# s-elkazdadi/ddp-pinocchio

Hardware: AMD Instinct MI355X
Metric: DDP iterations/sec (fwd+bwd sweep), Talos nq=38 T=200 (higher is better)
Workload: dtype f64

## Files before the change

ddp_pinocchio_amd/csrc/lin_static.hip:

```cpp
#include <float.h>
#include <math.h>
#include <stdlib.h>

#include <type_traits>
#include <utility>

#include "internal.h"
#include "lin_common.h"
#include "rbd.h"

#ifndef DEV_NO_EMIT
#define DEV_NO_EMIT 0
#endif
namespace {

struct TopoTalos38 {
  static constexpr int N = 38;
  static constexpr int parent[N] = {-1, 0, 1, 2, 3, 4,
                                    5, 6, 7, 8, 9, 10,
                                    5, 12, 13, 14, 15, 16,
                                    5, 18,
                                    19, 20, 21, 22, 23, 24, 25, 26,
                                    19, 28, 29, 30, 31, 32, 33, 34,
                                    19, 36};
  static constexpr int prismatic[N] = {1, 1, 1, 0, 0, 0, 0, 0, 0, 0, 0, 0, 0, 0, 0, 0, 0, 0, 0,
                                       0, 0, 0, 0, 0, 0, 0, 0, 0, 0, 0, 0, 0, 0, 0, 0, 0, 0, 0};
};

struct TopoChain6 {
  static constexpr int N = 6;
  static constexpr int parent[N] = {-1, 0, 1, 2, 3, 4};
  static constexpr int prismatic[N] = {0, 0, 0, 0, 0, 0};
};

}
#include "topo_extra.h"
namespace {

template <class T> constexpr bool has_child(int k) {
  for (int c = k + 1; c < T::N; ++c) if (T::parent[c] == k) return true;
  return false;
}
template <class T> constexpr int largest_child(int k) {
  int r = -1;
  for (int c = k + 1; c < T::N; ++c) if (T::parent[c] == k) r = c;
  return r;
}
template <class T> constexpr bool first_contrib(int k) { return T::parent[k] >= 0 && largest_child<T>(T::parent[k]) == k; }

template <class T>
bool topo_matches(const DevModel& m) {
  if (m.kind != DDP_HIP_MODEL_TREE || m.nv != T::N) return false;
  for (int i = 0; i < T::N; ++i)
    if (m.parent[i] != T::parent[i] || (m.jtype[i] == DDP_HIP_JOINT_PRISMATIC) != (T::prismatic[i] != 0)) return false;
  return true;
}

template <class T>
struct TauState {
  double acc[T::N][6];
  double uu[T::N];
};

template <class T, int K, int QS>
__device__ __forceinline__ void tau_up(const DevModel& m, const double* __restrict__ qc, const double* __restrict__ vc,
                                       double tauK, TauState<T>& s) {
  constexpr int o = T::prismatic[K] ? 3 : 0;
  const double* E = qc + K * QS;
  const double* r = E + 9;
  const double* U = E + 12;
  const double dinv = E[18];
  const double* pA0 = vc + K * rbd::VC_STRIDE + 6;
  const double* Iac = vc + K * rbd::VC_STRIDE + 12;
  const double* a = m.axis[K];
  double pAi[6];
  if constexpr (has_child<T>(K)) {
#pragma unroll
    for (int k = 0; k < 6; ++k) pAi[k] = s.acc[K][k];
  } else {
#pragma unroll
    for (int k = 0; k < 6; ++k) pAi[k] = pA0[k];
  }
  double sp = 0;
#pragma unroll
  for (int k = 0; k < 3; ++k) sp += a[k] * pAi[o + k];
  const double ui = tauK - sp;
  s.uu[K] = ui;
  constexpr int par = T::parent[K];
  if constexpr (par >= 0) {
    double pa[6], fp[6];
#pragma unroll
    for (int k = 0; k < 6; ++k) pa[k] = pAi[k] + Iac[k] + U[k] * (ui * dinv);
    rbd::xform_force_T(E, r, pa, fp);
    if constexpr (first_contrib<T>(K)) {
      const double* pp0 = vc + par * rbd::VC_STRIDE + 6;
#pragma unroll
      for (int k = 0; k < 6; ++k) s.acc[par][k] = pp0[k] + fp[k];
    } else {
#pragma unroll
      for (int k = 0; k < 6; ++k) s.acc[par][k] += fp[k];
    }
  }
  if constexpr (QS == rbd::QC_STRIDE || (K % 2) == 0) __builtin_amdgcn_sched_barrier(0);
}

template <class T, int K, int QS>
__device__ __forceinline__ void tau_down(const DevModel& m, const double* __restrict__ qc, const double* __restrict__ vc,
                                         TauState<T>& s) {
  constexpr int o = T::prismatic[K] ? 3 : 0;
  const double* E = qc + K * QS;
  const double* r = E + 9;
  const double* U = E + 12;
  const double dinv = E[18];
  const double* cb = vc + K * rbd::VC_STRIDE;
  double ap[6];
  constexpr int par = T::parent[K];
  if constexpr (par >= 0) rbd::xform_motion(E, r, s.acc[par], ap);
  else {
    const double a0[6] = {0, 0, 0, -m.gravity[0], -m.gravity[1], -m.gravity[2]};
    rbd::xform_motion(E, r, a0, ap);
  }
  double sum = 0;
#pragma unroll
  for (int k = 0; k < 6; ++k) { ap[k] += cb[k]; sum += U[k] * ap[k]; }
  const double qd = (s.uu[K] - sum) * dinv;
  s.uu[K] = qd;
  if constexpr (has_child<T>(K)) {
    const double* a = m.axis[K];
#pragma unroll
    for (int k = 0; k < 6; ++k) s.acc[K][k] = ap[k];
    s.acc[K][o] += a[0] * qd; s.acc[K][o + 1] += a[1] * qd; s.acc[K][o + 2] += a[2] * qd;
  }
  if constexpr (QS == rbd::QC_STRIDE || (K % 2) == 0) __builtin_amdgcn_sched_barrier(0);
}

template <class T, int QS, class TauFn, int... Ks>
__device__ __forceinline__ void tau_up_all(const DevModel& m, const double* __restrict__ qc, const double* __restrict__ vc, TauFn tau,
                                           TauState<T>& s, std::integer_sequence<int, Ks...>) {
  (tau_up<T, T::N - 1 - Ks, QS>(m, qc, vc, tau(T::N - 1 - Ks), s), ...);
}
template <class T, int QS, int HI, class TauFn, int... Ks>
__device__ __forceinline__ void tau_up_range(const DevModel& m, const double* __restrict__ qc, const double* __restrict__ vc, TauFn tau,
                                             TauState<T>& s, std::integer_sequence<int, Ks...>) {
  (tau_up<T, HI - Ks, QS>(m, qc, vc, tau(HI - Ks), s), ...);
}
template <class T, int QS, int... Ks>
__device__ __forceinline__ void tau_down_all(const DevModel& m, const double* __restrict__ qc, const double* __restrict__ vc,
                                             TauState<T>& s, std::integer_sequence<int, Ks...>) {
  (tau_down<T, Ks, QS>(m, qc, vc, s), ...);
}

constexpr int PS = 20;
template <int NV>
__device__ __forceinline__ void stage_placements(double* sp, const double* __restrict__ qc, int lane) {
  for (int idx = lane; idx < NV * 19; idx += LBS) {
    const int K = idx / 19, e = idx - K * 19;
    sp[K * PS + e] = qc[K * rbd::QC_STRIDE + e];
  }
}

template <int BYTES>
__device__ __forceinline__ unsigned int warm_block(const double* base, int lane) {
  typedef unsigned int u4 __attribute__((ext_vector_type(4)));
  const char* b = reinterpret_cast<const char*>(base);
  unsigned int sink = 0;
#pragma unroll
  for (int off = 0; off < BYTES; off += LBS * 16) {
    int o = off + lane * 16;
    o = o < BYTES - 16 ? o : BYTES - 16;
    const u4 v = *reinterpret_cast<const u4*>(b + o);
    sink ^= v.x ^ v.y ^ v.z ^ v.w;
  }
  return sink;
}

template <class T> constexpr bool parents_at_least(int from, int lo) {
  for (int k = from; k < T::N; ++k) if (T::parent[k] < lo) return false;
  return true;
}
template <class T> constexpr int stage_split() {
  for (int kh = T::N / 2; kh > 0; --kh) if (parents_at_least<T>(kh + 1, kh)) return kh;
  return 0;
}

template <int NV, int K0, int K1, bool WITH_V = true>
struct StageRegs {
  static constexpr int NPW = (K1 - K0) * 19, NVW = WITH_V ? (K1 - K0) * rbd::VC_STRIDE : 0;
  static constexpr int CP = (NPW + LBS - 1) / LBS, CV = (NVW + LBS - 1) / LBS;
  double rp[CP], rv[CV > 0 ? CV : 1];
  __device__ __forceinline__ void load(const double* __restrict__ qc, const double* __restrict__ vc, int lane) {
#pragma unroll
    for (int c = 0; c < CP; ++c) {
      int idx = c * LBS + lane;
      idx = idx < NPW ? idx : NPW - 1;
      const int K = K0 + idx / 19, e = idx % 19;
      rp[c] = qc[K * rbd::QC_STRIDE + e];
    }
#pragma unroll
    for (int c = 0; c < CV; ++c) {
      int idx = c * LBS + lane;
      idx = idx < NVW ? idx : NVW - 1;
      rv[c] = vc[K0 * rbd::VC_STRIDE + idx];
    }
  }
  __device__ __forceinline__ void park(double* sp, double* sv, int lane) const {
#pragma unroll
    for (int c = 0; c < CP; ++c) {
      int idx = c * LBS + lane;
      idx = idx < NPW ? idx : NPW - 1;
      const int K = K0 + idx / 19, e = idx % 19;
      sp[K * PS + e] = rp[c];
    }
#pragma unroll
    for (int c = 0; c < CV; ++c) {
      int idx = c * LBS + lane;
      idx = idx < NVW ? idx : NVW - 1;
      sv[K0 * rbd::VC_STRIDE + idx] = rv[c];
    }
  }
};

__device__ __forceinline__ void tri_index(int64_t q, int Wd, int& ii, int& jj) {
  int a = (int)floor(((2.0 * Wd - 1.0) - sqrt((2.0 * Wd - 1.0) * (2.0 * Wd - 1.0) - 8.0 * (double)q)) * 0.5);
  if (a < 0) a = 0;
  while ((int64_t)a * (2 * Wd - a - 1) / 2 > q) --a;
  while ((int64_t)(a + 1) * (2 * Wd - a - 2) / 2 <= q) ++a;
  ii = a;
  jj = (int)(q - (int64_t)a * (2 * Wd - a - 1) / 2) + a + 1;
}

template <int NV, int NP = LBS>
struct OutStage {
  double qdd[NP * (NV + 1)];
  int pij[NP];
};

template <int NV, int NP>
__device__ __forceinline__ void offdiag_emit(const LinParams& p, OutStage<NV, NP>& S, bool valid, int i, int j, int64_t bt,
                                             const double* __restrict__ xg, double dt, int pass = 0) {
  constexpr int n = 2 * NV, mm = NV;
  constexpr int RW = 16, NJ = (n + RW - 1) / RW, GRP = LBS / RW, PPG = NP / GRP, NB = NP == LBS ? 2 : 1;
  static_assert(PPG % NB == 0, "points per group");
  const double eps = sqrt(sqrt(DBL_EPSILON));
  const double eps2 = eps * eps;
  const int lane = threadIdx.x;
  if (lane / NP == pass) S.pij[lane % NP] = i | (j << 8) | ((valid ? 1 : 0) << 16);
  double* const fxx = p.fxx + bt * n * n * n;
  double* const fux = p.fux + bt * n * mm * n;
  double* const fuu = p.fuu + bt * n * mm * mm;
  const double* const fxb = p.fx + bt * n * n;
  const double* const fub = p.fu + bt * n * mm;
  __syncthreads();
  const int kk = lane % RW, grp = lane / RW;
  const double* f0 = p.f_val + bt * n;
  double f0k[NJ], xk[NJ], xvk[NJ];
#pragma unroll
  for (int jx = 0; jx < NJ; ++jx) {
    const int k = kk + RW * jx;
    const int kc = k < n ? k : n - 1;
    f0k[jx] = f0[kc];
    xk[jx] = xg[kc];
    xvk[jx] = kc < NV ? xg[NV + kc] : 0.0;
  }
  if (DEV_NO_EMIT) return;
  for (int pt = 0; pt < PPG; pt += NB) {
    double a1[NB][NJ], a2[NB][NJ], d1[NB][NJ], d2[NB][NJ];
    double* o0[NB];
    double* o1[NB];
    int ie[NB], je[NB], ee[NB];
#pragma unroll
    for (int u = 0; u < NB; ++u) {
      const int e = (pt + u) * GRP + grp;
      ee[u] = e;
      const int pk = S.pij[e];
      const int i1 = pk & 255, j1 = (pk >> 8) & 255;
      ie[u] = i1;
      je[u] = j1;
      const bool at_x_1 = i1 < n, at_x_2 = j1 < n;
      const int idx_1 = at_x_1 ? i1 : i1 - n, idx_2 = at_x_2 ? j1 : j1 - n;
      double* tensor;
      int L;
      if (at_x_1) { if (at_x_2) { tensor = fxx; L = n; } else { tensor = fux; L = mm; } }
      else { tensor = fuu; L = mm; }
      o0[u] = (pk >> 16) ? tensor + (int64_t)idx_2 * n + (int64_t)idx_1 * n * L : nullptr;
      o1[u] = ((pk >> 16) && at_x_1 == at_x_2 && !p.skip_qv_mirror) ? tensor + (int64_t)idx_1 * n + (int64_t)idx_2 * n * L : nullptr;
      if (o0[u]) {
        const double* q0 = at_x_1 ? fxb + (int64_t)idx_1 * n : fub + (int64_t)idx_1 * n;
        const double* q1 = at_x_2 ? fxb + (int64_t)idx_2 * n : fub + (int64_t)idx_2 * n;
        const double* q2 = at_x_1 ? fxx + (int64_t)idx_1 * n + (int64_t)idx_1 * n * n : fuu + (int64_t)idx_1 * n + (int64_t)idx_1 * n * mm;
        const double* q3 = at_x_2 ? fxx + (int64_t)idx_2 * n + (int64_t)idx_2 * n * n : fuu + (int64_t)idx_2 * n + (int64_t)idx_2 * n * mm;
#pragma unroll
        for (int jx = 0; jx < NJ; ++jx) {
          const int k = kk + RW * jx;
          const int kc = k < n ? k : n - 1;
          a1[u][jx] = q0[kc]; a2[u][jx] = q1[kc]; d1[u][jx] = q2[kc]; d2[u][jx] = q3[kc];
        }
      }
    }
#pragma unroll
    for (int u = 0; u < NB; ++u) {
      if (!o0[u]) continue;
#pragma unroll
      for (int jx = 0; jx < NJ; ++jx) {
        const int k = kk + RW * jx;
        if (k >= n) continue;
        if (p.skip_top && k < NV && !((ie[u] < n && ie[u] % NV == k) || (je[u] < n && je[u] % NV == k))) continue;
        double xs = k == ie[u] ? xk[jx] + eps : xk[jx];
        if (k == je[u]) xs = xs + eps;
        double fv;
        if (k < NV) {
          double xv = (NV + k) == ie[u] ? xvk[jx] + eps : xvk[jx];
          if (NV + k == je[u]) xv = xv + eps;
          const double vo = dt * xv;
          fv = xs + vo;
        } else {
          fv = xs + S.qdd[ee[u] * (NV + 1) + (k - NV)] * dt;
        }
        double df = fv - f0k[jx];
        df -= eps * a1[u][jx];
        df -= eps * a2[u][jx];
        df *= 2;
        const double val = 0.5 * (df / eps2 - d1[u][jx] - d2[u][jx]);
        o0[u][k] = val;
        if (o1[u]) o1[u][k] = val;
      }
    }
  }
}

template <int NV>
struct RowStage {
  double q[(NV + 2) * (NV + 1)];
};

template <int NV, bool DIAG_ROW, class ST>
__device__ __forceinline__ void rowblock_emit(const ST& S, int lane, int i, int jb, double* __restrict__ out, double* __restrict__ mirror,
                                              int64_t mstride, const double* __restrict__ a2, const double* __restrict__ d2, int64_t dstride,
                                              double dt, const double* __restrict__ f0g, const double* __restrict__ a1g,
                                              double* __restrict__ d1g, const double* __restrict__ xg, bool skip_top = false) {
  constexpr int n = 2 * NV, RW = 16, NJ = (n + RW - 1) / RW, CG = LBS / RW, NIT = (NV + CG - 1) / CG;
  const int r1 = i % NV;
  const double eps = sqrt(sqrt(DBL_EPSILON));
  const double eps2 = eps * eps;
  const int kk = lane % RW, cg = lane / RW;
  double xk[NJ], xvk[NJ], f0k[NJ], a1k[NJ], d1k[NJ];
#pragma unroll
  for (int j = 0; j < NJ; ++j) {
    const int k = kk + RW * j;
    const int kc = k < n ? k : n - 1;
    f0k[j] = f0g[kc];
    a1k[j] = a1g[kc];
    double x = xg[kc];
    if (kc == i) x = x + eps;
    xk[j] = x;
    double xv = xg[kc < NV ? NV + kc : kc];
    if (NV + kc == i) xv = xv + eps;
    xvk[j] = xv;
    if constexpr (DIAG_ROW) {
      double fv;
      if (kc < NV) {
        const double vo = dt * xv;
        fv = x + vo;
      } else {
        fv = x + S.q[NV * (NV + 1) + (kc - NV)] * dt;
      }
      double df = fv - f0k[j];
      df -= eps * a1k[j];
      df *= 2;
      const double dd = df / eps2;
      d1k[j] = dd;
      if (cg == 0 && k < n && !(skip_top && k < NV && k != r1)) d1g[k] = dd;
    } else {
      d1k[j] = d1g[kc];
    }
  }
  double va2[2][NJ], vd2[2][NJ];
  auto fetch = [&](int it, double (&A)[NJ], double (&D)[NJ]) {
    const int c = it * CG + cg;
    const int cc = c < NV ? c : NV - 1;
#pragma unroll
    for (int j = 0; j < NJ; ++j) {
      const int k = kk + RW * j;
      const int kc = k < n ? k : n - 1;
      A[j] = a2[kc + cc * n];
      D[j] = d2[kc + cc * dstride];
    }
  };
  auto form = [&](int it, const double (&A)[NJ], const double (&D)[NJ]) {
    const int c = it * CG + cg;
    const bool cv = c < NV;
    const int cc = cv ? c : NV - 1;
    const int jp = jb + cc;
#pragma unroll
    for (int j = 0; j < NJ; ++j) {
      const int k = kk + RW * j;
      if (!(cv && k < n)) continue;
      if (skip_top && k < NV && k != r1 && !(jp < n && jp % NV == k)) continue;
      double x = xk[j];
      if (k == jp) x = x + eps;
      double fv;
      if (k < NV) {
        double xv = xvk[j];
        if (NV + k == jp) xv = xv + eps;
        const double vo = dt * xv;
        fv = x + vo;
      } else {
        fv = x + S.q[cc * (NV + 1) + (k - NV)] * dt;
      }
      double df = fv - f0k[j];
      df -= eps * a1k[j];
      df -= eps * A[j];
      df *= 2;
      const double val = 0.5 * (df / eps2 - d1k[j] - D[j]);
      out[k + c * n] = val;
      if (mirror) mirror[k + c * mstride] = val;
    }
  };
  if (DEV_NO_EMIT) return;
  fetch(0, va2[0], vd2[0]);
  for (int it = 0; it < NIT; it += 2) {
    if (it + 1 < NIT) fetch(it + 1, va2[1], vd2[1]);
    form(it, va2[0], vd2[0]);
    if (it + 1 < NIT) {
      if (it + 2 < NIT) fetch(it + 2, va2[0], vd2[0]);
      form(it + 1, va2[1], vd2[1]);
    }
  }
}

template <class T, bool ROWS>
__global__ __launch_bounds__(LBS, ROWS ? 1 : 3) void lin_static_tau_kernel(LinParams p) {
  constexpr int nv = T::N, n = 2 * nv;
  constexpr int TRI = nv * (nv - 1) / 2, GU = (TRI + LBS - 1) / LBS, G = ROWS ? 2 * nv : GU;
  const int64_t bt = blockIdx.x / G;
  const int g = (int)(blockIdx.x % G) + (ROWS ? 0 : 2 * nv);
  const int lane = threadIdx.x;
  const int64_t Tn = p.d.T;
  const int b = (int)(bt / Tn);
  const int64_t t = bt % Tn;
  const DevModel& m = *p.model;
  int i, j, cfg, vcfg;
  bool valid;
  if (g < nv) { i = g; j = n + lane; cfg = 1 + g; vcfg = nv + 1 + g; valid = lane < nv; }
  else if (g < 2 * nv) { i = g; j = n + lane; cfg = 0; vcfg = 1 + (g - nv); valid = lane < nv; }
  else {
    const int pid = (g - 2 * nv) * LBS + lane;
    valid = pid < TRI;
    tri_index(valid ? pid : 0, nv, i, j);
    i += n; j += n; cfg = 0; vcfg = 0;
  }
  double eps = sqrt(sqrt(DBL_EPSILON));
  const double* __restrict__ qc = p.qcache + (bt * (nv + 1) + cfg) * (int64_t)nv * rbd::QC_STRIDE;
  const double* __restrict__ vc = p.vcache + (bt * (2 * nv + 1) + vcfg) * (int64_t)nv * rbd::VC_STRIDE;
  const double* __restrict__ xg = p.x + ((int64_t)b * (Tn + 1) + t) * n;
  const double* __restrict__ ug = p.u + ((int64_t)b * Tn + t) * nv;
  const int iu = i - n, ju = j - n;
  __shared__ union TauLds { double P[ROWS ? nv * PS + nv * rbd::VC_STRIDE : 1]; RowStage<nv> S; } s_lds;
  double* s_P = s_lds.P;
  unsigned int w = 0;
  double* s_V = s_P + nv * PS;
  constexpr int KH = ROWS ? stage_split<T>() : 0;
  StageRegs<nv, 0, (ROWS && KH > 0) ? KH : 1> lower;
  if constexpr (ROWS) {
    StageRegs<nv, KH, nv> upper;
    upper.load(qc, vc, lane);
    lower.load(qc, vc, lane);
    upper.park(s_P, s_V, lane);
    rbd::coop_sync<true>();
  } else {
    w = warm_block<nv * rbd::VC_STRIDE * 8>(vc, lane);
    w ^= warm_block<nv * rbd::QC_STRIDE * 8>(qc, lane);
  }
  if (w == 0x7fc01234u) eps = 0.0;
  TauState<T> s;
  auto tau = [&](int k) { double v = ug[k]; if (k == iu) v = v + eps; if (k == ju) v = v + eps; return v; };
  if constexpr (ROWS) {
    static_assert(!ROWS || parents_at_least<T>(KH + 1, KH), "the first half of the pass must not reach below record KH");
    tau_up_range<T, PS, nv - 1>(m, s_P, s_V, tau, s, std::make_integer_sequence<int, nv - 1 - KH>{});
    lower.park(s_P, s_V, lane);
    rbd::coop_sync<true>();
    tau_up_range<T, PS, KH>(m, s_P, s_V, tau, s, std::make_integer_sequence<int, KH + 1>{});
    tau_down_all<T, PS>(m, s_P, s_V, s, std::make_integer_sequence<int, nv>{});
  } else {
    tau_up_all<T, rbd::QC_STRIDE>(m, qc, vc, tau, s, std::make_integer_sequence<int, nv>{});
    tau_down_all<T, rbd::QC_STRIDE>(m, qc, vc, s, std::make_integer_sequence<int, nv>{});
  }
  __builtin_amdgcn_sched_barrier(0);
  typedef __attribute__((address_space(4))) const LinParams* kernarg_t;
  const kernarg_t kp = (kernarg_t)__builtin_amdgcn_kernarg_segment_ptr();
  if constexpr (ROWS) {
    RowStage<nv>& S = s_lds.S;
    const int mm = nv;
    __syncthreads();
    const int row = lane <= nv ? lane : nv + 1;
#pragma unroll
    for (int k = 0; k < nv; ++k) S.q[row * (nv + 1) + k] = s.uu[k];
    __syncthreads();
    rowblock_emit<nv, true>(S, lane, i, n, kp->fux + bt * n * mm * n + (int64_t)i * n * mm, nullptr, 0, kp->fu + bt * n * mm,
                            kp->fuu + bt * n * mm * mm, (int64_t)n + (int64_t)n * mm, m.dt, kp->f_val + bt * n,
                            kp->fx + bt * n * n + (int64_t)i * n, kp->fxx + bt * n * n * n + (int64_t)i * n + (int64_t)i * n * n, xg, kp->skip_top != 0);
  } else {
    __shared__ OutStage<nv, LBS / 2> S;
    LinParams po;
    po.f_val = kp->f_val; po.fx = kp->fx; po.fu = kp->fu; po.fxx = kp->fxx; po.fux = kp->fux; po.fuu = kp->fuu; po.skip_qv_mirror = kp->skip_qv_mirror; po.skip_top = kp->skip_top;
    const double dt = m.dt;
#pragma unroll 1
    for (int pass = 0; pass < 2; ++pass) {
      if (pass) __syncthreads();
      if (lane / (LBS / 2) == pass) {
#pragma unroll
        for (int k = 0; k < nv; ++k) S.qdd[(lane % (LBS / 2)) * (nv + 1) + k] = s.uu[k];
      }
      offdiag_emit<nv, LBS / 2>(po, S, valid, i, j, bt, xg, dt, pass);
    }
  }
}

template <class T> constexpr int n_children(int k) {
  int c = 0;
  for (int j = k + 1; j < T::N; ++j) if (T::parent[j] == k) ++c;
  return c;
}
template <class T> constexpr bool chain_start(int k) { return T::parent[k] < 0 || T::parent[k] != k - 1 || n_children<T>(T::parent[k]) > 1; }
template <class T> constexpr bool chain_end(int k) { return k == T::N - 1 || chain_start<T>(k + 1); }
template <class T> constexpr int chain_first(int k) { while (!chain_start<T>(k)) --k; return k; }
template <class T> constexpr int max_chain() {
  int best = 1;
  for (int k = 0; k < T::N; ++k)
    if (chain_end<T>(k)) { const int len = k - chain_first<T>(k) + 1; if (len > best) best = len; }
  return best;
}

template <class T>
struct VelState {
  double vel[T::N][6];
  double acc[T::N][6];
  double uu[T::N];
};

template <int UQS_, int QS_ = rbd::QC_STRIDE>
struct VelCtx {
  static constexpr int UQS = UQS_;
  static constexpr int QS = QS_;
  const DevModel* m;
  const double* qp;
  const double* __restrict__ qc;
  const double* __restrict__ xg;
  const double* __restrict__ ug;
  double* uq;
  int i, j;
  double eps;
  template <int K> __device__ __forceinline__ const double* er(double*) const { return qp + K * QS; }
  template <int K> __device__ __forceinline__ const double* er_down(double* b) const { return er<K>(b); }
  template <int K> __device__ __forceinline__ const double* ud() const { return qp + K * QS + 12; }
  template <int K> __device__ __forceinline__ void ia_cb(const double*, const double* cb, double* Iac) const { rbd::sym6_mv(qc + K * rbd::QC_STRIDE + 19, cb, Iac); }
  template <int K> __device__ __forceinline__ const double* ud_down() const { return ud<K>(); }
};

template <int NV, class C>
__device__ __forceinline__ double lane_v(const C& c, int K) {
  double v = c.xg[NV + K];
  if (NV + K == c.i) v = v + c.eps;
  if (NV + K == c.j) v = v + c.eps;
  return v;
}

template <class T, int K, class C>
__device__ __forceinline__ void joint_vel(const C& c, const double* vel_par, double* vel) {
  constexpr int o = T::prismatic[K] ? 3 : 0;
  double Pb[12];
  const double* E = c.template er<K>(Pb);
  const double* r = E + 9;
  const double* a = c.m->axis[K];
  const double vK = lane_v<T::N>(c, K);
  double vJ[6] = {0, 0, 0, 0, 0, 0};
  vJ[o] = a[0] * vK; vJ[o + 1] = a[1] * vK; vJ[o + 2] = a[2] * vK;
  if constexpr (T::parent[K] >= 0) rbd::xform_motion(E, r, vel_par, vel);
  else {
#pragma unroll
    for (int k = 0; k < 6; ++k) vel[k] = 0.0;
  }
#pragma unroll
  for (int k = 0; k < 6; ++k) vel[k] += vJ[k];
}
template <class T, int K, class C>
__device__ __forceinline__ void vel_from_root(const C& c, double* vel) {
  if constexpr (T::parent[K] >= 0) {
    double vp[6];
    vel_from_root<T, T::parent[K]>(c, vp);
    joint_vel<T, K>(c, vp, vel);
  } else {
    joint_vel<T, K>(c, nullptr, vel);
  }
}
template <class T, int K, class C>
__device__ __forceinline__ void bias_force0(const C& c, const double* vel, double* pA) {
  double Iv[6];
  rbd::sym6_mv(c.m->I6[K], vel, Iv);
  rbd::crf(vel, Iv, pA);
}

template <class T, int K, int E, class C>
__device__ __forceinline__ void chain_down(const C& c, VelState<T>& s) {
  if constexpr (T::parent[K] >= 0) joint_vel<T, K>(c, s.vel[T::parent[K]], s.vel[K]);
  else joint_vel<T, K>(c, nullptr, s.vel[K]);
  __builtin_amdgcn_sched_barrier(0);
  if constexpr (K < E) chain_down<T, K + 1, E>(c, s);
}

template <class T, int K, int F, class C>
__device__ __forceinline__ void chain_up(const C& c, VelState<T>& s) {
  constexpr int o = T::prismatic[K] ? 3 : 0;
  double Pb[12];
  const double* E = c.template er<K>(Pb);
  const double* r = E + 9;
  const double* U = c.template ud<K>();
  const double dinv = U[6];
  const double* a = c.m->axis[K];
  double pAi[6];
  if constexpr (has_child<T>(K)) {
#pragma unroll
    for (int k = 0; k < 6; ++k) pAi[k] = s.acc[K][k];
  } else {
    bias_force0<T, K>(c, s.vel[K], pAi);
  }
  double sp = 0;
#pragma unroll
  for (int k = 0; k < 3; ++k) sp += a[k] * pAi[o + k];
  const double ui = c.ug[K] - sp;
  if constexpr (C::UQS == 0) s.uu[K] = ui; else c.uq[K * C::UQS] = ui;
  constexpr int par = T::parent[K];
  if constexpr (par >= 0) {
    const double vK = lane_v<T::N>(c, K);
    double vJ[6] = {0, 0, 0, 0, 0, 0}, cb[6], pa[6], Iac[6], fp[6];
    vJ[o] = a[0] * vK; vJ[o + 1] = a[1] * vK; vJ[o + 2] = a[2] * vK;
    rbd::crm(s.vel[K], vJ, cb);
    c.template ia_cb<K>(U, cb, Iac);
#pragma unroll
    for (int k = 0; k < 6; ++k) pa[k] = pAi[k] + Iac[k] + U[k] * (ui * dinv);
    rbd::xform_force_T(E, r, pa, fp);
    if constexpr (first_contrib<T>(K)) {
      double p0[6];
      bias_force0<T, par>(c, s.vel[par], p0);
#pragma unroll
      for (int k = 0; k < 6; ++k) s.acc[par][k] = p0[k] + fp[k];
    } else {
#pragma unroll
      for (int k = 0; k < 6; ++k) s.acc[par][k] += fp[k];
    }
  }
  __builtin_amdgcn_sched_barrier(0);
  if constexpr (K > F) chain_up<T, K - 1, F>(c, s);
}

template <class T, int K, class C>
__device__ __forceinline__ void chain_at(const C& c, VelState<T>& s) {
  if constexpr (chain_end<T>(K)) {
    constexpr int F = chain_first<T>(K), P = T::parent[F];
    if constexpr (P >= 0) {
      if constexpr (first_contrib<T>(F) && n_children<T>(P) > 1) vel_from_root<T, P>(c, s.vel[P]);
    }
    chain_down<T, F, K>(c, s);
    chain_up<T, K, F>(c, s);
  }
}
template <class T, class C, int... Ks>
__device__ __forceinline__ void vel_up_all(const C& c, VelState<T>& s, std::integer_sequence<int, Ks...>) {
  (chain_at<T, T::N - 1 - Ks>(c, s), ...);
}

template <class T, int K, class C>
__device__ __forceinline__ void vel_down(const C& c, VelState<T>& s) {
  constexpr int o = T::prismatic[K] ? 3 : 0;
  constexpr int par = T::parent[K];
  double Pb[12];
  const double* E = c.template er_down<K>(Pb);
  const double* r = E + 9;
  const double* U = c.template ud_down<K>();
  const double dinv = U[6];
  const double* a = c.m->axis[K];
  const double vK = lane_v<T::N>(c, K);
  double vJ[6] = {0, 0, 0, 0, 0, 0}, vel[6], cb[6], ap[6];
  vJ[o] = a[0] * vK; vJ[o + 1] = a[1] * vK; vJ[o + 2] = a[2] * vK;
  if constexpr (par >= 0) {
    rbd::xform_motion(E, r, s.vel[par], vel);
    rbd::xform_motion(E, r, s.acc[par], ap);
  } else {
    const double a0[6] = {0, 0, 0, -c.m->gravity[0], -c.m->gravity[1], -c.m->gravity[2]};
#pragma unroll
    for (int k = 0; k < 6; ++k) vel[k] = 0.0;
    rbd::xform_motion(E, r, a0, ap);
  }
#pragma unroll
  for (int k = 0; k < 6; ++k) vel[k] += vJ[k];
  rbd::crm(vel, vJ, cb);
  double sum = 0;
#pragma unroll
  for (int k = 0; k < 6; ++k) { ap[k] += cb[k]; sum += U[k] * ap[k]; }
  double ui;
  if constexpr (C::UQS == 0) ui = s.uu[K]; else ui = c.uq[K * C::UQS];
  const double qd = (ui - sum) * dinv;
  if constexpr (C::UQS == 0) s.uu[K] = qd; else c.uq[K * C::UQS] = qd;
  if constexpr (has_child<T>(K)) {
#pragma unroll
    for (int k = 0; k < 6; ++k) { s.vel[K][k] = vel[k]; s.acc[K][k] = ap[k]; }
    s.acc[K][o] += a[0] * qd; s.acc[K][o + 1] += a[1] * qd; s.acc[K][o + 2] += a[2] * qd;
  }
  __builtin_amdgcn_sched_barrier(0);
}
template <class T, class C, int... Ks>
__device__ __forceinline__ void vel_down_all(const C& c, VelState<T>& s, std::integer_sequence<int, Ks...>) {
  (vel_down<T, Ks>(c, s), ...);
}

template <class T, bool ROWS>
__global__ __launch_bounds__(LBS, ROWS ? 3 : 1) void lin_static_vel_kernel(LinParams p) {
  constexpr int nv = T::N, n = 2 * nv;
  constexpr int TRI = nv * (nv - 1) / 2, GU = (TRI + LBS - 1) / LBS, G = ROWS ? nv : GU;
  const int64_t bt = blockIdx.x / G;
  const int g = (int)(blockIdx.x % G);
  const int lane = threadIdx.x;
  const int64_t Tn = p.d.T;
  const int b = (int)(bt / Tn);
  const int64_t t = bt % Tn;
  int i, j, cfg;
  bool valid;
  if (ROWS) { i = g; j = nv + lane; cfg = 1 + g; valid = lane < nv; }
  else {
    const int pid = g * LBS + lane;
    valid = pid < TRI;
    tri_index(valid ? pid : 0, nv, i, j);
    i += nv; j += nv; cfg = 0;
  }
  using Stage = typename std::conditional<ROWS, RowStage<nv>, OutStage<nv>>::type;
  __shared__ union VelLds { Stage S; double P[ROWS ? nv * rbd::QC_STRIDE : 1]; } s_lds;
  Stage& S = s_lds.S;
  double* s_P = s_lds.P;
  VelCtx<ROWS ? 0 : 1, rbd::QC_STRIDE> c;
  c.m = p.model;
  c.qc = p.qcache + (bt * (nv + 1) + cfg) * (int64_t)nv * rbd::QC_STRIDE;
  c.qp = ROWS ? s_P : c.qc;
  c.xg = p.x + ((int64_t)b * (Tn + 1) + t) * n;
  c.ug = p.u + ((int64_t)b * Tn + t) * nv;
  c.i = i; c.j = j;
  c.eps = sqrt(sqrt(DBL_EPSILON));
  if constexpr (ROWS) c.uq = nullptr;
  else c.uq = &S.qdd[lane * (nv + 1)];
  if constexpr (ROWS) {
    constexpr int NW = nv * rbd::QC_STRIDE, CW = (NW + LBS - 1) / LBS;
    double rq[CW];
#pragma unroll
    for (int r = 0; r < CW; ++r) { const int idx = r * LBS + lane; rq[r] = c.qc[idx < NW ? idx : NW - 1]; }
#pragma unroll
    for (int r = 0; r < CW; ++r) { const int idx = r * LBS + lane; s_P[idx < NW ? idx : NW - 1] = rq[r]; }
    c.qc = s_P;
    rbd::coop_sync<true>();
  } else {
    const unsigned int w = warm_block<nv * rbd::QC_STRIDE * 8>(c.qc, lane);
    if (w == 0x7fc01234u) c.eps = 0.0;
  }
  VelState<T> s;
  vel_up_all<T>(c, s, std::make_integer_sequence<int, nv>{});
  vel_down_all<T>(c, s, std::make_integer_sequence<int, nv>{});
  __builtin_amdgcn_sched_barrier(0);
  typedef __attribute__((address_space(4))) const LinParams* kernarg_t;
  const kernarg_t kp = (kernarg_t)__builtin_amdgcn_kernarg_segment_ptr();
  const double dt = c.m->dt;
  if constexpr (ROWS) {
    double* fxx = kp->fxx + bt * n * n * n;
    const double* fxb = kp->fx + bt * n * n;
    __syncthreads();
    const int row = valid ? lane : nv;
#pragma unroll
    for (int k = 0; k < nv; ++k) S.q[row * (nv + 1) + k] = s.uu[k];
    __syncthreads();
    rowblock_emit<nv, false>(S, lane, i, nv, fxx + (int64_t)nv * n + (int64_t)i * n * n,
                             kp->skip_qv_mirror ? nullptr : fxx + (int64_t)i * n + (int64_t)nv * n * n, (int64_t)n * n,
                             fxb + (int64_t)nv * n, fxx + (int64_t)nv * n + (int64_t)nv * n * n, (int64_t)n + (int64_t)n * n, dt,
                             kp->f_val + bt * n, fxb + (int64_t)i * n, fxx + (int64_t)i * n + (int64_t)i * n * n, c.xg, kp->skip_top != 0);
  } else {
    LinParams po;
    po.f_val = kp->f_val; po.fx = kp->fx; po.fu = kp->fu; po.fxx = kp->fxx; po.fux = kp->fux; po.fuu = kp->fuu; po.skip_qv_mirror = kp->skip_qv_mirror; po.skip_top = kp->skip_top;
    offdiag_emit<nv, LBS>(po, S, valid, i, j, bt, c.xg, dt);
  }
}

constexpr int WS_PER_JOINT = 8;

template <class T>
struct CfgState {
  double vel[T::N][6];
  double accP[T::N][6];
  double accI[T::N][21];
  double w[2][WS_PER_JOINT];
};

struct CfgCtx {
  const DevModel* __restrict__ m;
  const double* __restrict__ qc0;
  const double* __restrict__ xg;
  const double* __restrict__ ug;
  double* __restrict__ W;
  double* lvel;
  int i, j;
  const double* own;
};

template <int K, int NV>
__device__ __forceinline__ void lane_placement(const CfgCtx& c, double* P) {
  const double* base = c.qc0 + K * rbd::QC_STRIDE;
  const double* pert = c.own ? c.own : c.qc0 + ((int64_t)(1 + K) * NV + K) * rbd::QC_STRIDE;
  const bool own = K == c.i || K == c.j;
#pragma unroll
  for (int e = 0; e < 12; ++e) P[e] = own ? pert[e] : base[e];
}

template <class T, int K>
__device__ __forceinline__ void cfg_joint_vel(const CfgCtx& c, const double* P, const double* vel_par, double* vel) {
  constexpr int o = T::prismatic[K] ? 3 : 0;
  const double* a = c.m->axis[K];
  const double vK = c.xg[T::N + K];
  double vJ[6] = {0, 0, 0, 0, 0, 0};
  vJ[o] = a[0] * vK; vJ[o + 1] = a[1] * vK; vJ[o + 2] = a[2] * vK;
  if constexpr (T::parent[K] >= 0) rbd::xform_motion(P, P + 9, vel_par, vel);
  else {
#pragma unroll
    for (int k = 0; k < 6; ++k) vel[k] = 0.0;
  }
#pragma unroll
  for (int k = 0; k < 6; ++k) vel[k] += vJ[k];
}
template <class T, int K>
__device__ __forceinline__ void cfg_vel_from_root(const CfgCtx& c, double* vel) {
  double P[12];
  lane_placement<K, T::N>(c, P);
  if constexpr (T::parent[K] >= 0) {
    double vp[6];
    cfg_vel_from_root<T, T::parent[K]>(c, vp);
    cfg_joint_vel<T, K>(c, P, vp, vel);
  } else {
    cfg_joint_vel<T, K>(c, P, nullptr, vel);
  }
}
template <int K>
__device__ __forceinline__ void cfg_bias_force0(const CfgCtx& c, const double* vel, double* pA) {
  double Iv[6];
  rbd::sym6_mv(c.m->I6[K], vel, Iv);
  rbd::crf(vel, Iv, pA);
}

template <class T, int K, int F, int E>
__device__ __forceinline__ void cfg_chain_down(const CfgCtx& c, CfgState<T>& s, double* cur) {
  double P[12], vel[6];
  lane_placement<K, T::N>(c, P);
  if constexpr (T::parent[K] >= 0) cfg_joint_vel<T, K>(c, P, cur, vel);
  else cfg_joint_vel<T, K>(c, P, nullptr, vel);
#pragma unroll
  for (int k = 0; k < 6; ++k) { cur[k] = vel[k]; c.lvel[((K - F) * 6 + k) * LBS] = vel[k]; }
  __builtin_amdgcn_sched_barrier(0);
  if constexpr (K < E) cfg_chain_down<T, K + 1, F, E>(c, s, cur);
}
template <class T, int K, int F>
__device__ __forceinline__ void chain_vel_load(const CfgCtx& c, const CfgState<T>& s, double* vel) {
  if constexpr (K >= F) {
#pragma unroll
    for (int k = 0; k < 6; ++k) vel[k] = c.lvel[((K - F) * 6 + k) * LBS];
  } else {
#pragma unroll
    for (int k = 0; k < 6; ++k) vel[k] = s.vel[K][k];
  }
}

template <class T, int K, int F>
__device__ __forceinline__ void cfg_chain_up(const CfgCtx& c, CfgState<T>& s) {
  constexpr int o = T::prismatic[K] ? 3 : 0;
  const double* a = c.m->axis[K];
  double IA[21], pAi[6], U[6], velK[6];
  chain_vel_load<T, K, F>(c, s, velK);
  if constexpr (has_child<T>(K)) {
#pragma unroll
    for (int k = 0; k < 21; ++k) IA[k] = s.accI[K][k];
#pragma unroll
    for (int k = 0; k < 6; ++k) pAi[k] = s.accP[K][k];
  } else {
#pragma unroll
    for (int k = 0; k < 21; ++k) IA[k] = c.m->I6[K][k];
    cfg_bias_force0<K>(c, velK, pAi);
  }
  double d = 0, sp = 0;
#pragma unroll
  for (int r = 0; r < 6; ++r) U[r] = IA[rbd::sidx(r, o)] * a[0] + IA[rbd::sidx(r, o + 1)] * a[1] + IA[rbd::sidx(r, o + 2)] * a[2];
#pragma unroll
  for (int k = 0; k < 3; ++k) { d += a[k] * U[o + k]; sp += a[k] * pAi[o + k]; }
  const double dinv = 1.0 / d;
  const double ui = c.ug[K] - sp;
#pragma unroll
  for (int k = 0; k < 6; ++k) c.W[(K * WS_PER_JOINT + k) * LBS] = U[k];
  c.W[(K * WS_PER_JOINT + 6) * LBS] = dinv;
  c.W[(K * WS_PER_JOINT + 7) * LBS] = ui;
  constexpr int par = T::parent[K];
  if constexpr (par >= 0) {
    double P[12], Ia[21], vJ[6] = {0, 0, 0, 0, 0, 0}, cb[6], pa[6], Iac[6], fp[6];
    lane_placement<K, T::N>(c, P);
    const double vK = c.xg[T::N + K];
    vJ[o] = a[0] * vK; vJ[o + 1] = a[1] * vK; vJ[o + 2] = a[2] * vK;
#pragma unroll
    for (int r = 0; r < 6; ++r)
#pragma unroll
      for (int cc = 0; cc <= r; ++cc) Ia[rbd::sidx(r, cc)] = IA[rbd::sidx(r, cc)] - U[r] * U[cc] * dinv;
    rbd::crm(velK, vJ, cb);
    rbd::sym6_mv(Ia, cb, Iac);
#pragma unroll
    for (int k = 0; k < 6; ++k) pa[k] = pAi[k] + Iac[k] + U[k] * (ui * dinv);
    if constexpr (first_contrib<T>(K)) {
      double velP[6];
      chain_vel_load<T, par, F>(c, s, velP);
#pragma unroll
      for (int k = 0; k < 21; ++k) s.accI[par][k] = c.m->I6[par][k];
      cfg_bias_force0<par>(c, velP, s.accP[par]);
    }
    rbd::add_xtix(P, P + 9, Ia, s.accI[par]);
    rbd::xform_force_T(P, P + 9, pa, fp);
#pragma unroll
    for (int k = 0; k < 6; ++k) s.accP[par][k] += fp[k];
  }
  __builtin_amdgcn_sched_barrier(0);
  if constexpr (K > F) cfg_chain_up<T, K - 1, F>(c, s);
}

template <class T, int K>
__device__ __forceinline__ void cfg_chain_at(const CfgCtx& c, CfgState<T>& s) {
  if constexpr (chain_end<T>(K)) {
    constexpr int F = chain_first<T>(K), P = T::parent[F];
    if constexpr (P >= 0) {
      if constexpr (first_contrib<T>(F) && n_children<T>(P) > 1) cfg_vel_from_root<T, P>(c, s.vel[P]);
    }
    double cur[6] = {0, 0, 0, 0, 0, 0};
    if constexpr (P >= 0) {
#pragma unroll
      for (int k = 0; k < 6; ++k) cur[k] = s.vel[P][k];
    }
    cfg_chain_down<T, F, F, K>(c, s, cur);
    cfg_chain_up<T, K, F>(c, s);
  }
}
template <class T, int... Ks>
__device__ __forceinline__ void cfg_up_all(const CfgCtx& c, CfgState<T>& s, std::integer_sequence<int, Ks...>) {
  (cfg_chain_at<T, T::N - 1 - Ks>(c, s), ...);
}

template <int STRIDE_>
struct CfgDownOut { double* uq; static constexpr int STRIDE = STRIDE_; };

template <class T, int K, class O>
__device__ __forceinline__ void cfg_down(const CfgCtx& c, CfgState<T>& s, const O& out) {
  constexpr int o = T::prismatic[K] ? 3 : 0;
  constexpr int par = T::parent[K];
  if constexpr (K + 1 < T::N) {
#pragma unroll
    for (int e = 0; e < WS_PER_JOINT; ++e) s.w[(K + 1) & 1][e] = c.W[((K + 1) * WS_PER_JOINT + e) * LBS];
  }
  const double* U = s.w[K & 1];
  const double dinv = s.w[K & 1][6], ui = s.w[K & 1][7];
  const double* a = c.m->axis[K];
  const double vK = c.xg[T::N + K];
  double P[12], vJ[6] = {0, 0, 0, 0, 0, 0}, vel[6], cb[6], ap[6];
  lane_placement<K, T::N>(c, P);
  vJ[o] = a[0] * vK; vJ[o + 1] = a[1] * vK; vJ[o + 2] = a[2] * vK;
  if constexpr (par >= 0) {
    rbd::xform_motion(P, P + 9, s.vel[par], vel);
    rbd::xform_motion(P, P + 9, s.accP[par], ap);
  } else {
    const double a0[6] = {0, 0, 0, -c.m->gravity[0], -c.m->gravity[1], -c.m->gravity[2]};
#pragma unroll
    for (int k = 0; k < 6; ++k) vel[k] = 0.0;
    rbd::xform_motion(P, P + 9, a0, ap);
  }
#pragma unroll
  for (int k = 0; k < 6; ++k) vel[k] += vJ[k];
  rbd::crm(vel, vJ, cb);
  double sum = 0;
#pragma unroll
  for (int k = 0; k < 6; ++k) { ap[k] += cb[k]; sum += U[k] * ap[k]; }
  const double qd = (ui - sum) * dinv;
  out.uq[K * (O::STRIDE == LBS ? LBS : 1)] = qd;
  if constexpr (has_child<T>(K)) {
#pragma unroll
    for (int k = 0; k < 6; ++k) { s.vel[K][k] = vel[k]; s.accP[K][k] = ap[k]; }
    s.accP[K][o] += a[0] * qd; s.accP[K][o + 1] += a[1] * qd; s.accP[K][o + 2] += a[2] * qd;
  }
  __builtin_amdgcn_sched_barrier(0);
}
template <class T, class O, int... Ks>
__device__ __forceinline__ void cfg_down_all(const CfgCtx& c, CfgState<T>& s, const O& out, std::integer_sequence<int, Ks...>) {
  (cfg_down<T, Ks>(c, s, out), ...);
}

template <class T>
__device__ __forceinline__ void cfg_setup(CfgCtx& c, const LinParams& p, const DevModel* __restrict__ model, const double* __restrict__ qcache,
                                          const double* __restrict__ xs, const double* __restrict__ us, double* __restrict__ ws,
                                          int64_t bt0, int64_t& bt, bool& valid) {
  constexpr int nv = T::N, n = 2 * nv;
  constexpr int TRI = nv * (nv - 1) / 2, GU = (TRI + LBS - 1) / LBS;
  bt = bt0 + blockIdx.x / GU;
  const int g = (int)(blockIdx.x % GU);
  const int lane = threadIdx.x;
  const int64_t Tn = p.d.T;
  const int b = (int)(bt / Tn);
  const int64_t t = bt % Tn;
  const int pid = g * LBS + lane;
  valid = pid < TRI;
  tri_index(valid ? pid : 0, nv, c.i, c.j);
  c.m = model;
  c.qc0 = qcache + (bt * (nv + 1)) * (int64_t)nv * rbd::QC_STRIDE;
  c.xg = xs + ((int64_t)b * (Tn + 1) + t) * n;
  c.ug = us + ((int64_t)b * Tn + t) * nv;
  c.W = ws + (int64_t)blockIdx.x * (nv * WS_PER_JOINT * LBS) + lane;
  c.own = nullptr;
}

template <class T>
__global__ __launch_bounds__(LBS) void lin_static_cfg_up_kernel(LinParams p, const DevModel* __restrict__ model, const double* __restrict__ qcache,
                                                                const double* __restrict__ xs, const double* __restrict__ us,
                                                                double* __restrict__ ws, int64_t bt0) {
  constexpr int nv = T::N;
  constexpr int MAXCH = max_chain<T>();
  __shared__ double s_vel[MAXCH * 6 * LBS];
  CfgCtx c;
  int64_t bt;
  bool valid;
  cfg_setup<T>(c, p, model, qcache, xs, us, ws, bt0, bt, valid);
  c.lvel = s_vel + threadIdx.x;
  CfgState<T> s;
  cfg_up_all<T>(c, s, std::make_integer_sequence<int, nv>{});
}

template <class T>
__global__ __launch_bounds__(LBS) void lin_static_cfg_down_kernel(LinParams p, const DevModel* __restrict__ model, const double* __restrict__ qcache,
                                                                  const double* __restrict__ xs, const double* __restrict__ us,
                                                                  double* __restrict__ ws, int64_t bt0) {
  constexpr int nv = T::N;
  __shared__ OutStage<nv> S;
  CfgCtx c;
  int64_t bt;
  bool valid;
  cfg_setup<T>(c, p, model, qcache, xs, us, ws, bt0, bt, valid);
  c.lvel = nullptr;
  CfgState<T> s;
#pragma unroll
  for (int e = 0; e < WS_PER_JOINT; ++e) s.w[0][e] = c.W[e * LBS];
  CfgDownOut<nv + 1> o{&S.qdd[threadIdx.x * (nv + 1)]};
  cfg_down_all<T>(c, s, o, std::make_integer_sequence<int, nv>{});
  __builtin_amdgcn_sched_barrier(0);
  typedef __attribute__((address_space(4))) const LinParams* kernarg_t;
  const kernarg_t kp = (kernarg_t)__builtin_amdgcn_kernarg_segment_ptr();
  LinParams po;
  po.f_val = kp->f_val; po.fx = kp->fx; po.fu = kp->fu; po.fxx = kp->fxx; po.fux = kp->fux; po.fuu = kp->fuu; po.skip_qv_mirror = kp->skip_qv_mirror; po.skip_top = kp->skip_top;
  offdiag_emit<nv, LBS>(po, S, valid, c.i, c.j, bt, c.xg, model->dt);
}

constexpr int SREC = 13;

template <class T>
struct SpineTab {
  static constexpr int N = T::N, TRI = N * (N - 1) / 2;
  static_assert(N >= 2 && N <= 64, "ancestor masks are 64 bits wide");
  unsigned long long mask[N];
  unsigned long long anc[N];
  int depth[N];
  int nrec;
  short pi[TRI], pj[TRI];
  short top[TRI];
  int rbase[TRI], rstride[TRI];
};
template <class T>
constexpr SpineTab<T> make_spine_tab() {
  SpineTab<T> t{};
  for (int k = 0; k < T::N; ++k)
    for (int a = T::parent[k]; a >= 0; a = T::parent[a]) { ++t.depth[k]; t.mask[a] |= 1ull << k; t.anc[k] |= 1ull << a; }
  int cnt[T::N + 2] = {}, start[T::N + 2] = {}, goff[T::N + 2] = {};
  for (int i = 0; i < T::N; ++i)
    for (int j = i + 1; j < T::N; ++j) {
      int a = T::parent[i];
      while (a >= 0 && !((t.mask[a] >> j) & 1)) a = T::parent[a];
      ++cnt[a + 1];
    }
// ... 656 lines not shown
```

Before: 682.8.

## Stage config caches through LDS in off-diagonal tau/vel kernels and halve output stage

The off-diagonal (non-ROWS) tau and velocity kernels now stage placement and velocity caches into shared memory with the cooperative load and park scheme the row kernels already used, replacing the global-memory warm-up reads and direct global accesses. The velocity kernel's output staging becomes a half-size two-pass buffer inside the LDS union, and its launch bound rises to allow two blocks per CU. The aim is to cut global-memory latency in the recursive passes and shrink the LDS footprint to improve occupancy. The cost is extra barriers, an extra emit pass, and LDS use shared across phases.

```diff
diff --git a/ddp_pinocchio_amd/csrc/lin_static.hip b/ddp_pinocchio_amd/csrc/lin_static.hip
--- a/ddp_pinocchio_amd/csrc/lin_static.hip
+++ b/ddp_pinocchio_amd/csrc/lin_static.hip
@@ -157,21 +157,6 @@
     const int K = idx / 19, e = idx - K * 19;
     sp[K * PS + e] = qc[K * rbd::QC_STRIDE + e];
   }
-}
-
-template <int BYTES>
-__device__ __forceinline__ unsigned int warm_block(const double* base, int lane) {
-  typedef unsigned int u4 __attribute__((ext_vector_type(4)));
-  const char* b = reinterpret_cast<const char*>(base);
-  unsigned int sink = 0;
-#pragma unroll
-  for (int off = 0; off < BYTES; off += LBS * 16) {
-    int o = off + lane * 16;
-    o = o < BYTES - 16 ? o : BYTES - 16;
-    const u4 v = *reinterpret_cast<const u4*>(b + o);
-    sink ^= v.x ^ v.y ^ v.z ^ v.w;
-  }
-  return sink;
 }
 
 template <class T> constexpr bool parents_at_least(int from, int lo) {
@@ -449,42 +434,32 @@
     tri_index(valid ? pid : 0, nv, i, j);
     i += n; j += n; cfg = 0; vcfg = 0;
   }
-  double eps = sqrt(sqrt(DBL_EPSILON));
+  const double eps = sqrt(sqrt(DBL_EPSILON));
   const double* __restrict__ qc = p.qcache + (bt * (nv + 1) + cfg) * (int64_t)nv * rbd::QC_STRIDE;
   const double* __restrict__ vc = p.vcache + (bt * (2 * nv + 1) + vcfg) * (int64_t)nv * rbd::VC_STRIDE;
   const double* __restrict__ xg = p.x + ((int64_t)b * (Tn + 1) + t) * n;
   const double* __restrict__ ug = p.u + ((int64_t)b * Tn + t) * nv;
   const int iu = i - n, ju = j - n;
-  __shared__ union TauLds { double P[ROWS ? nv * PS + nv * rbd::VC_STRIDE : 1]; RowStage<nv> S; } s_lds;
+  __shared__ union TauLds { double P[nv * PS + nv * rbd::VC_STRIDE]; RowStage<nv> S; OutStage<nv, LBS / 2> O; } s_lds;
   double* s_P = s_lds.P;
-  unsigned int w = 0;
   double* s_V = s_P + nv * PS;
-  constexpr int KH = ROWS ? stage_split<T>() : 0;
-  StageRegs<nv, 0, (ROWS && KH > 0) ? KH : 1> lower;
-  if constexpr (ROWS) {
+  constexpr int KH = stage_split<T>();
+  StageRegs<nv, 0, (KH > 0) ? KH : 1> lower;
+  {
     StageRegs<nv, KH, nv> upper;
     upper.load(qc, vc, lane);
     lower.load(qc, vc, lane);
     upper.park(s_P, s_V, lane);
     rbd::coop_sync<true>();
-  } else {
-    w = warm_block<nv * rbd::VC_STRIDE * 8>(vc, lane);
-    w ^= warm_block<nv * rbd::QC_STRIDE * 8>(qc, lane);
-  }
-  if (w == 0x7fc01234u) eps = 0.0;
+  }
   TauState<T> s;
   auto tau = [&](int k) { double v = ug[k]; if (k == iu) v = v + eps; if (k == ju) v = v + eps; return v; };
-  if constexpr (ROWS) {
-    static_assert(!ROWS || parents_at_least<T>(KH + 1, KH), "the first half of the pass must not reach below record KH");
-    tau_up_range<T, PS, nv - 1>(m, s_P, s_V, tau, s, std::make_integer_sequence<int, nv - 1 - KH>{});
-    lower.park(s_P, s_V, lane);
-    rbd::coop_sync<true>();
-    tau_up_range<T, PS, KH>(m, s_P, s_V, tau, s, std::make_integer_sequence<int, KH + 1>{});
-    tau_down_all<T, PS>(m, s_P, s_V, s, std::make_integer_sequence<int, nv>{});
-  } else {
-    tau_up_all<T, rbd::QC_STRIDE>(m, qc, vc, tau, s, std::make_integer_sequence<int, nv>{});
-    tau_down_all<T, rbd::QC_STRIDE>(m, qc, vc, s, std::make_integer_sequence<int, nv>{});
-  }
+  static_assert(parents_at_least<T>(KH + 1, KH), "the first half of the pass must not reach below record KH");
+  tau_up_range<T, PS, nv - 1>(m, s_P, s_V, tau, s, std::make_integer_sequence<int, nv - 1 - KH>{});
+  lower.park(s_P, s_V, lane);
+  rbd::coop_sync<true>();
+  tau_up_range<T, PS, KH>(m, s_P, s_V, tau, s, std::make_integer_sequence<int, KH + 1>{});
+  tau_down_all<T, PS>(m, s_P, s_V, s, std::make_integer_sequence<int, nv>{});
   __builtin_amdgcn_sched_barrier(0);
   typedef __attribute__((address_space(4))) const LinParams* kernarg_t;
   const kernarg_t kp = (kernarg_t)__builtin_amdgcn_kernarg_segment_ptr();
@@ -500,10 +475,11 @@
                             kp->fuu + bt * n * mm * mm, (int64_t)n + (int64_t)n * mm, m.dt, kp->f_val + bt * n,
                             kp->fx + bt * n * n + (int64_t)i * n, kp->fxx + bt * n * n * n + (int64_t)i * n + (int64_t)i * n * n, xg, kp->skip_top != 0);
   } else {
-    __shared__ OutStage<nv, LBS / 2> S;
+    OutStage<nv, LBS / 2>& S = s_lds.O;
     LinParams po;
     po.f_val = kp->f_val; po.fx = kp->fx; po.fu = kp->fu; po.fxx = kp->fxx; po.fux = kp->fux; po.fuu = kp->fuu; po.skip_qv_mirror = kp->skip_qv_mirror; po.skip_top = kp->skip_top;
     const double dt = m.dt;
+    __syncthreads();
 #pragma unroll 1
     for (int pass = 0; pass < 2; ++pass) {
       if (pass) __syncthreads();
@@ -714,7 +690,7 @@
 }
 
 template <class T, bool ROWS>
-__global__ __launch_bounds__(LBS, ROWS ? 3 : 1) void lin_static_vel_kernel(LinParams p) {
+__global__ __launch_bounds__(LBS, ROWS ? 3 : 2) void lin_static_vel_kernel(LinParams p) {
   constexpr int nv = T::N, n = 2 * nv;
   constexpr int TRI = nv * (nv - 1) / 2, GU = (TRI + LBS - 1) / LBS, G = ROWS ? nv : GU;
   const int64_t bt = blockIdx.x / G;
@@ -732,21 +708,21 @@
     tri_index(valid ? pid : 0, nv, i, j);
     i += nv; j += nv; cfg = 0;
   }
-  using Stage = typename std::conditional<ROWS, RowStage<nv>, OutStage<nv>>::type;
-  __shared__ union VelLds { Stage S; double P[ROWS ? nv * rbd::QC_STRIDE : 1]; } s_lds;
+  struct PairStage { OutStage<nv, LBS / 2> O; double spare[nv + 1]; };
+  using Stage = typename std::conditional<ROWS, RowStage<nv>, PairStage>::type;
+  __shared__ union VelLds { Stage S; double P[nv * rbd::QC_STRIDE]; } s_lds;
   Stage& S = s_lds.S;
   double* s_P = s_lds.P;
-  VelCtx<ROWS ? 0 : 1, rbd::QC_STRIDE> c;
+  VelCtx<0, rbd::QC_STRIDE> c;
   c.m = p.model;
   c.qc = p.qcache + (bt * (nv + 1) + cfg) * (int64_t)nv * rbd::QC_STRIDE;
-  c.qp = ROWS ? s_P : c.qc;
+  c.qp = s_P;
   c.xg = p.x + ((int64_t)b * (Tn + 1) + t) * n;
   c.ug = p.u + ((int64_t)b * Tn + t) * nv;
   c.i = i; c.j = j;
   c.eps = sqrt(sqrt(DBL_EPSILON));
-  if constexpr (ROWS) c.uq = nullptr;
-  else c.uq = &S.qdd[lane * (nv + 1)];
-  if constexpr (ROWS) {
+  c.uq = nullptr;
+  {
     constexpr int NW = nv * rbd::QC_STRIDE, CW = (NW + LBS - 1) / LBS;
     double rq[CW];
 #pragma unroll
@@ -755,9 +731,6 @@
     for (int r = 0; r < CW; ++r) { const int idx = r * LBS + lane; s_P[idx < NW ? idx : NW - 1] = rq[r]; }
     c.qc = s_P;
     rbd::coop_sync<true>();
-  } else {
-    const unsigned int w = warm_block<nv * rbd::QC_STRIDE * 8>(c.qc, lane);
-    if (w == 0x7fc01234u) c.eps = 0.0;
   }
   VelState<T> s;
   vel_up_all<T>(c, s, std::make_integer_sequence<int, nv>{});
@@ -779,9 +752,25 @@
                              fxb + (int64_t)nv * n, fxx + (int64_t)nv * n + (int64_t)nv * n * n, (int64_t)n + (int64_t)n * n, dt,
                              kp->f_val + bt * n, fxb + (int64_t)i * n, fxx + (int64_t)i * n + (int64_t)i * n * n, c.xg, kp->skip_top != 0);
   } else {
+    constexpr int NP = LBS / 2;
     LinParams po;
     po.f_val = kp->f_val; po.fx = kp->fx; po.fu = kp->fu; po.fxx = kp->fxx; po.fux = kp->fux; po.fuu = kp->fuu; po.skip_qv_mirror = kp->skip_qv_mirror; po.skip_top = kp->skip_top;
-    offdiag_emit<nv, LBS>(po, S, valid, i, j, bt, c.xg, dt);
+    __syncthreads();
+    double* const own = &S.O.qdd[(lane % NP) * (nv + 1)];
+    double* const row = lane < NP ? own : S.spare;
+#pragma unroll
+    for (int k = 0; k < nv; ++k) row[k] = s.uu[k];
+#pragma unroll 1
+    for (int pass = 0; pass < 2; ++pass) {
+      if (pass) {
+        __syncthreads();
+        if (lane >= NP) {
+#pragma unroll
+          for (int k = 0; k < nv; ++k) own[k] = s.uu[k];
+        }
+      }
+      offdiag_emit<nv, NP>(po, S.O, valid, i, j, bt, c.xg, dt, pass);
+    }
   }
 }
 
```

Result: faster. 711.0, median of 6 (+4.1%).
